# francescobrigante/Audio-Style-Transfer

Measured on AMD Instinct MI355X. Metric: audio-seconds/sec/node (train step, 4s@22.05kHz pairs), higher is better.
Workload: dtype bf16; 1 GPU; configs[1]: batch=8 4 s clips per GPU (S=2, x=(B,S,2,287,597)), full train2 step: STFT + CQT front-end from resident waveforms, encoders+decoder+discriminator, all losses, D and G phases, grad clip, Adam; global_batch=8, parallelism=dp1, hip_graph=True, dp_semantics=per-rank BN and batch-coupled losses

## Files before the change

### audio-style-transfer_amd/csrc/wgrad.hip

```cpp
#include "gemm_common.h"
#include <limits.h>

namespace {

#ifdef AST_STAMPS
__device__ unsigned long long ast_wg_stamps[4096 * 8];
__device__ long long ast_wg_phase[4096 * 4];
#define WG_STAMP(k) do { if (threadIdx.x == 0 && tix < 4096) ast_wg_stamps[tix * 8 + (k)] = (k) >= 6 ? wall_clock64() : __builtin_readcyclecounter(); } while (0)
#else
#define WG_STAMP(k) do { } while (0)
#endif
template <int BMW, int NCT, int RT, int CTW, typename WtOf>
__device__ __forceinline__ void flush_tile_rows(const f32x4 (&acc)[RT][CTW], float* tile, float* dw, const ast_gather_t& g, const int cd0,
                                                const int col0, const int ncols, const int wave, const int lane, WtOf wt_of, const int mode) {
  constexpr int BNW = NCT * 16;
  const int li = lane & 15, gq = lane >> 4;
  if (mode == 0) {
#pragma unroll
    for (int j = 0; j < CTW; ++j) {
      const int ct = wave + 4 * j;
      const int col = col0 + ct * 16 + li;
      if (ct >= NCT || col >= ncols) continue;
      const int t = col / g.Cs, c = col - t * g.Cs;
      const int wtc = wt_of(t);
#pragma unroll
      for (int i = 0; i < RT; ++i)
#pragma unroll
        for (int r = 0; r < 4; ++r) {
          const int cd = cd0 + i * 16 + gq * 4 + r;
          if (cd < g.Cd) unsafeAtomicAdd(dw + ((size_t)cd * g.wtaps + wtc) * g.Cs + c, acc[i][j][r]);
        }
    }
    return;
  }
  __syncthreads();
#pragma unroll
  for (int j = 0; j < CTW; ++j) {
    const int ct = wave + 4 * j;
    if (ct < NCT) {
#pragma unroll
      for (int i = 0; i < RT; ++i)
#pragma unroll
        for (int r = 0; r < 4; ++r) tile[(i * 16 + gq * 4 + r) * BNW + ct * 16 + li] = acc[i][j][r];
    }
  }
  __syncthreads();
#pragma unroll
  for (int cc = 0; cc < BNW / 64; ++cc) {
    const int col = col0 + cc * 64 + lane;
    if (col >= ncols) continue;
    const int t = col / g.Cs, c = col - t * g.Cs;
    float* dcol = dw + (size_t)wt_of(t) * g.Cs + c;
    if (mode == 2) {
      for (int row = wave; row < BMW; row += 4) {
        const int cd = cd0 + row;
        if (cd < g.Cd) dcol[(size_t)cd * g.wtaps * g.Cs] = tile[row * BNW + cc * 64 + lane];
      }
    } else {
      for (int row = wave; row < BMW; row += 4) {
        const int cd = cd0 + row;
        if (cd < g.Cd) unsafeAtomicAdd(dcol + (size_t)cd * g.wtaps * g.Cs, tile[row * BNW + cc * 64 + lane]);
      }
    }
  }
}

struct WgradFlush {
  enum Mode { Atomic = 0, AtomicLds = 1, Slab = 2 } mode;
  int copies;
  long stride;
  int* slices_out;
};
inline WgradFlush::Mode wg_atomic_mode() { return env_flag("AST_WGRAD_FLUSH_LDS", false) ? WgradFlush::AtomicLds : WgradFlush::Atomic; }
inline int wg_flush_arg(const WgradFlush& f) { return f.copies | ((int)f.mode << 16); }
inline int wg_slice_cap(const WgradFlush& f) { return f.mode == WgradFlush::Slab ? f.copies : INT_MAX; }
inline void wg_report_slices(const WgradFlush& f, int slices) { if (f.slices_out) *f.slices_out = slices; }
inline int wg_target_knob(int fallback) { return env_int("AST_WGRAD_WG_TARGET", fallback); }
inline int wg_pg_knob(int fallback) { return env_int("AST_WGRAD_PG", fallback); }

struct PixelSlices { int nsplit, pps, grid; };
inline PixelSlices plan_pixel_slices(int P, int k_unit, int min_trips, int tiles, int want, int cap) {
  const int min_px = min_trips * k_unit;
  int nsplit = std::min(std::max(1, std::min((P + min_px - 1) / min_px, want)), cap);
  int pps = (P + nsplit - 1) / nsplit;
  pps = (pps + k_unit - 1) / k_unit * k_unit;
  nsplit = (P + pps - 1) / pps;
  return {nsplit, pps, (tiles * nsplit + 7) / 8 * 8};
}
template <typename T> struct WgradCfg;
template <> struct WgradCfg<bf16_t> { static constexpr int BKP = 64, PAD = 16; };
template <> struct WgradCfg<float> { static constexpr int BKP = 32, PAD = 16; };

template <typename T, int BMW, int NCT, int PG, bool SLAB>
__global__ __launch_bounds__(256 * PG) void wgrad_kernel(const T* __restrict__ dy, const T* __restrict__ src,
                                                     float* __restrict__ dw, const ast_gather_t g,
                                                     const int P, const int pps, const unsigned dy_bytes,
                                                     const unsigned src_bytes, const float rcp_hw, const float rcp_w,
                                                     const int gx, const int gy, const int gz, const int nrep, const long rep_stride) {
  constexpr int E = 16 / sizeof(T), ES = sizeof(T);
  constexpr int BKP = WgradCfg<T>::BKP, PAD = WgradCfg<T>::PAD;
  constexpr int BNW = NCT * 16;
  constexpr int TPR = 256 / BKP;
  constexpr int CPX = BNW / E, CPY = BMW / E;
  constexpr int NXI = (CPX + TPR - 1) / TPR, NYI = (CPY + TPR - 1) / TPR;
  constexpr int PX = BNW + PAD, PY = BMW + PAD;
  constexpr bool SWZ = sizeof(T) == 2 && (CPX % 2 == 0) && (CPY % 2 == 0);
  constexpr int RT = BMW / 16;
  constexpr int CTW = (NCT + 3) / 4;
  constexpr unsigned OOB = 0x80000000u;
  extern __shared__ __attribute__((aligned(16))) unsigned char wl_all[];
  constexpr int GROUP_BYTES = (int)sizeof(T) * BKP * (PY + PX);
  constexpr int RED = PG > 1 ? RT * CTW * 256 * 16 : 0;
  constexpr int TILE = BMW * BNW * 4;
  constexpr int TAP_OFF = std::max(std::max(PG * GROUP_BYTES, RED), TILE);
  const int pg = PG > 1 ? __builtin_amdgcn_readfirstlane(threadIdx.x >> 8) : 0;
  unsigned char* wl = wl_all + pg * GROUP_BYTES;
  T* Ys = reinterpret_cast<T*>(wl);
  T* Xs = Ys + BKP * PY;
  int* taptab = reinterpret_cast<int*>(wl_all + TAP_OFF);

  const int tid = threadIdx.x & 255, lane = tid & 63, wave = tid >> 6;
  const int chunk = gridDim.x >> 3;
  const int tix = (blockIdx.x & 7) * chunk + (blockIdx.x >> 3);
  if (tix >= gx * gy * gz) return;
  WG_STAMP(0); WG_STAMP(7);
  const int bx = tix / (gz * gy), bz = (tix / gy) % gz, by = tix % gy;
  const int cd0 = bx * BMW, col0 = by * BNW;
  const int ncols = g.ntaps * g.Cs;
  const int HWm = g.Hm * g.Wm;
  const int p_begin = bz * pps, p_end = min(P, p_begin + pps);
  const __amdgpu_buffer_rsrc_t dyR = __builtin_amdgcn_make_buffer_rsrc((void*)dy, 0, dy_bytes, 0x00020000);
  const __amdgpu_buffer_rsrc_t srcR = __builtin_amdgcn_make_buffer_rsrc((void*)src, 0, src_bytes, 0x00020000);
#pragma unroll
  for (int t = 0; t < AST_MAX_TAPS; ++t)
    if ((int)threadIdx.x == t) taptab[t] = g.tap[t];
  __syncthreads();

  const int lrow = tid / TPR, tq = tid % TPR;
  int xdelta[NXI], xdh[NXI], xdw[NXI];
#pragma unroll
  for (int i = 0; i < NXI; ++i) {
    const int ch = tq + TPR * i, col = col0 + ch * E;
    xdelta[i] = 0; xdh[i] = 1 << 20; xdw[i] = 0;
    if (ch < CPX && col < ncols) {
      const int t = col / g.Cs, c = col - t * g.Cs;
      int dh, dw_, wt;
      decode_tap(taptab[t], dh, dw_, wt);
      xdh[i] = dh; xdw[i] = dw_;
      xdelta[i] = ((dh * g.Ws + dw_) * g.Cs + c) * ES;
    }
  }
  u32x4 yreg[NYI], xreg[NXI];
  auto load_tile = [&](int p0) __attribute__((always_inline)) {
    const int p = p0 + lrow;
    const bool pv = p < p_end;
    const int pp = pv ? p : 0;
#pragma unroll
    for (int i = 0; i < NYI; ++i) {
      const int ch = tq + TPR * i, cd = cd0 + ch * E;
      const bool ok = pv && ch < CPY && cd < g.Cd;
      yreg[i] = __builtin_amdgcn_raw_buffer_load_b128(dyR, ok ? (unsigned)((pp * g.Cd + cd) * ES) : OOB, 0, 0);
    }
    const int n = fdiv(pp, HWm, rcp_hw), rem = pp - n * HWm;
    const int hm = fdiv(rem, g.Wm, rcp_w), wq = rem - hm * g.Wm;
    const int hs0 = pv ? hm * g.sh + g.oh : -(1 << 21), ws0 = wq * g.sw + g.ow;
    const int base = (((n * g.Hs + hs0) * g.Ws + ws0) * g.Cs) * ES;
#pragma unroll
    for (int i = 0; i < NXI; ++i) {
      const bool ok = (unsigned)(hs0 + xdh[i]) < (unsigned)g.Hs && (unsigned)(ws0 + xdw[i]) < (unsigned)g.Ws;
      xreg[i] = __builtin_amdgcn_raw_buffer_load_b128(srcR, ok ? (unsigned)(base + xdelta[i]) : OOB, 0, 0);
    }
  };
  auto store_tile = [&]() __attribute__((always_inline)) {
    const int sw = SWZ ? ((lrow >> 3) & 1) << 1 : 0;
#pragma unroll
    for (int i = 0; i < NYI; ++i) {
      const int ch = tq + TPR * i;
      if (ch < CPY) *reinterpret_cast<u32x4*>(Ys + lrow * PY + (ch ^ sw) * E) = yreg[i];
    }
#pragma unroll
    for (int i = 0; i < NXI; ++i) {
      const int ch = tq + TPR * i;
      if (ch < CPX) *reinterpret_cast<u32x4*>(Xs + lrow * PX + (ch ^ sw) * E) = xreg[i];
    }
  };

  f32x4 acc[RT][CTW];
#pragma unroll
  for (int i = 0; i < RT; ++i)
#pragma unroll
    for (int j = 0; j < CTW; ++j) acc[i][j] = f32x4{0.f, 0.f, 0.f, 0.f};

  const int li = lane & 15, gq = lane >> 4;
  const int nk_all = (p_end - p_begin + BKP - 1) / BKP;
  const int nk = (nk_all + PG - 1) / PG;
  if (nk > 0) load_tile(p_begin + pg * BKP);
  WG_STAMP(1);
#ifdef AST_STAMPS
  long long ph[5] = {0, 0, 0, 0, 0};
#define WG_PH(i) do { const long long t_ = __builtin_readcyclecounter(); ph[i] += t_ - tph; tph = t_; } while (0)
  long long tph = __builtin_readcyclecounter();
#else
#define WG_PH(i) do { } while (0)
#endif
  for (int kt = 0; kt < nk; ++kt) {
    store_tile();
    WG_PH(0);
    __syncthreads();
    WG_PH(1);
    if (kt + 1 < nk) load_tile(p_begin + ((kt + 1) * PG + pg) * BKP);
    WG_PH(2);
    if constexpr (sizeof(T) == 2) {
      typedef __attribute__((address_space(3))) bf16x4 lds_b4;
      const int q = li >> 2, pcol = (li & 3) * 4;
#pragma unroll
      for (int ks = 0; ks < BKP / 32; ++ks) {
        const int r_lo = ks * 32 + 8 * gq + q;
        const int sx = SWZ ? (gq & 1) << 4 : 0;
        bf16x8 af[RT];
#pragma unroll
        for (int i = 0; i < RT; ++i) {
          const bf16x4 lo = __builtin_amdgcn_ds_read_tr16_b64_v4bf16((lds_b4*)(Ys + r_lo * PY + ((i * 16) ^ sx) + pcol));
          const bf16x4 hi = __builtin_amdgcn_ds_read_tr16_b64_v4bf16((lds_b4*)(Ys + (r_lo + 4) * PY + ((i * 16) ^ sx) + pcol));
          af[i] = bf16x8{lo[0], lo[1], lo[2], lo[3], hi[0], hi[1], hi[2], hi[3]};
        }
#pragma unroll
        for (int j = 0; j < CTW; ++j) {
          const int ct = wave + 4 * j;
          if (ct < NCT) {
            const bf16x4 lo = __builtin_amdgcn_ds_read_tr16_b64_v4bf16((lds_b4*)(Xs + r_lo * PX + ((ct * 16) ^ sx) + pcol));
            const bf16x4 hi = __builtin_amdgcn_ds_read_tr16_b64_v4bf16((lds_b4*)(Xs + (r_lo + 4) * PX + ((ct * 16) ^ sx) + pcol));
            const bf16x8 bf = bf16x8{lo[0], lo[1], lo[2], lo[3], hi[0], hi[1], hi[2], hi[3]};
#pragma unroll
            for (int i = 0; i < RT; ++i) acc[i][j] = __builtin_amdgcn_mfma_f32_16x16x32_bf16(af[i], bf, acc[i][j], 0, 0, 0);
          }
        }
      }
    } else {
#pragma unroll
      for (int s4 = 0; s4 < BKP / 4; ++s4) {
        float af[RT];
#pragma unroll
        for (int i = 0; i < RT; ++i) af[i] = Ys[(4 * s4 + gq) * PY + i * 16 + li];
#pragma unroll
        for (int j = 0; j < CTW; ++j) {
          const int ct = wave + 4 * j;
          if (ct < NCT) {
            const float bf = Xs[(4 * s4 + gq) * PX + ct * 16 + li];
#pragma unroll
            for (int i = 0; i < RT; ++i) acc[i][j] = __builtin_amdgcn_mfma_f32_16x16x4f32(af[i], bf, acc[i][j], 0, 0, 0);
          }
        }
      }
    }
    WG_PH(3);
    __syncthreads();
    WG_PH(4);
  }
#ifdef AST_STAMPS
  if (threadIdx.x == 0 && tix < 4096) { ast_wg_stamps[tix * 8 + 5] = (unsigned long long)((ph[0] << 32) | (ph[1] & 0xffffffffll)); ast_wg_phase[tix * 4 + 0] = ph[2]; ast_wg_phase[tix * 4 + 1] = ph[3]; ast_wg_phase[tix * 4 + 2] = ph[4]; ast_wg_phase[tix * 4 + 3] = nk; }
#endif

  WG_STAMP(2);
  if constexpr (PG > 1) {
    f32x4* red = reinterpret_cast<f32x4*>(wl_all);
#pragma unroll
    for (int src_g = 1; src_g < PG; ++src_g) {
      __syncthreads();
      if (pg == src_g) {
#pragma unroll
        for (int i = 0; i < RT; ++i)
#pragma unroll
          for (int j = 0; j < CTW; ++j) red[(i * CTW + j) * 256 + tid] = acc[i][j];
      }
      __syncthreads();
      if (pg == 0) {
#pragma unroll
        for (int i = 0; i < RT; ++i)
#pragma unroll
          for (int j = 0; j < CTW; ++j) {
            const f32x4 t = red[(i * CTW + j) * 256 + tid];
            acc[i][j][0] += t[0]; acc[i][j][1] += t[1]; acc[i][j][2] += t[2]; acc[i][j][3] += t[3];
          }
      }
    }
    if (pg > 0) return;
  }
  WG_STAMP(3);
  dw += (size_t)(bz % (nrep & 0xffff)) * rep_stride;
  flush_tile_rows<BMW, NCT, RT, CTW>(acc, reinterpret_cast<float*>(wl_all), dw, g, cd0, col0, ncols, wave, lane,
                                     [&](int t) { return taptab[t] >> 16; }, SLAB ? 2 : (nrep >> 16) & 3);
#ifdef AST_STAMPS
  asm volatile("s_waitcnt vmcnt(0)" ::: "memory");
#endif
  WG_STAMP(4); WG_STAMP(6);
}
#ifdef AST_STAMPS
extern "C" int ast_debug_read_wg_stamps(unsigned long long* host, int n) {
  return (int)hipMemcpyFromSymbol(host, HIP_SYMBOL(ast_wg_stamps), (size_t)n * 8 * sizeof(unsigned long long));
}
extern "C" int ast_debug_read_wg_phases(long long* host, int n) {
  return (int)hipMemcpyFromSymbol(host, HIP_SYMBOL(ast_wg_phase), (size_t)n * 4 * sizeof(long long));
}
// ... 406 lines not shown
#pragma unroll
        for (int i = 0; i < RT; ++i) {
          const bf16x4 lo = __builtin_amdgcn_ds_read_tr16_b64_v4bf16((lds_b4*)(Ys + p_lo * PY + i * 16 + pcol));
          const bf16x4 hi = __builtin_amdgcn_ds_read_tr16_b64_v4bf16((lds_b4*)(Ys + p_hi * PY + i * 16 + pcol));
          af[i] = bf16x8{lo[0], lo[1], lo[2], lo[3], hi[0], hi[1], hi[2], hi[3]};
        }
#pragma unroll
        for (int j = 0; j < CTW; ++j) {
          if (wave + 4 * j < NCT) {
            const bf16x4 lo = __builtin_amdgcn_ds_read_tr16_b64_v4bf16((lds_b4*)(Xp + x_lo + coloff[j]));
            const bf16x4 hi = __builtin_amdgcn_ds_read_tr16_b64_v4bf16((lds_b4*)(Xp + x_hi + coloff[j]));
            const bf16x8 bf = bf16x8{lo[0], lo[1], lo[2], lo[3], hi[0], hi[1], hi[2], hi[3]};
#pragma unroll
            for (int i = 0; i < RT; ++i) acc[i][j] = __builtin_amdgcn_mfma_f32_16x16x32_bf16(af[i], bf, acc[i][j], 0, 0, 0);
          }
        }
      }
    } else {
#pragma unroll 4
      for (int s4 = 0; s4 < MT / 4; ++s4) {
        const int p = 4 * s4 + gq;
        const int xo = (((p >> 4) * g.sh) * PW + (p & 15) * g.sw) * PPX;
        float af[RT];
#pragma unroll
        for (int i = 0; i < RT; ++i) af[i] = Ys[p * PY + i * 16 + li];
#pragma unroll
        for (int j = 0; j < CTW; ++j) {
          if (wave + 4 * j < NCT) {
            const float bf = colok[j] ? Xp[xo + coloff[j]] : 0.f;
#pragma unroll
            for (int i = 0; i < RT; ++i) acc[i][j] = __builtin_amdgcn_mfma_f32_16x16x4f32(af[i], bf, acc[i][j], 0, 0, 0);
          }
        }
      }
    }
    __syncthreads();
  }

  if constexpr (PG > 1) {
    f32x4* red = reinterpret_cast<f32x4*>(wl_all);
#pragma unroll
    for (int src_g = 1; src_g < PG; ++src_g) {
      __syncthreads();
      if (pg == src_g) {
#pragma unroll
        for (int i = 0; i < RT; ++i)
#pragma unroll
          for (int j = 0; j < CTW; ++j) red[(i * CTW + j) * 256 + tid] = acc[i][j];
      }
      __syncthreads();
      if (pg == 0) {
#pragma unroll
        for (int i = 0; i < RT; ++i)
#pragma unroll
          for (int j = 0; j < CTW; ++j) {
            const f32x4 t = red[(i * CTW + j) * 256 + tid];
            acc[i][j][0] += t[0]; acc[i][j][1] += t[1]; acc[i][j][2] += t[2]; acc[i][j][3] += t[3];
          }
      }
    }
    if (pg > 0) return;
  }
  dw += (size_t)(blockIdx.z % (nrep & 0xffff)) * rep_stride;
  flush_tile_rows<BMW, NCT, RT, CTW>(acc, reinterpret_cast<float*>(wl_all), dw, g, cd0, col0, ncols, wave, lane,
                                     [&](int t) { return taptab[16 + t]; }, SLAB ? 2 : (nrep >> 16) & 3);
}

bool plan_wgrad_halo(const ast_gather_t& g, int dtype, int nct, int bmw, WHaloPlan& hp) {
  if (g.ntaps < 2 || g.Cd > env_int("AST_WGRAD_HALO_MAXCD", 32)) return false;
  const int E = dtype == AST_BF16 ? 8 : 4, ES = dtype == AST_BF16 ? 2 : 4;
  int dhmin = 64, dhmax = -64, dwmin = 64, dwmax = -64;
  for (int t = 0; t < g.ntaps; ++t) {
    const int dh = (g.tap[t] & 255) - 64, dw = ((g.tap[t] >> 8) & 255) - 64;
    dhmin = std::min(dhmin, dh); dhmax = std::max(dhmax, dh); dwmin = std::min(dwmin, dw); dwmax = std::max(dwmax, dw);
  }
  hp.dhmin = dhmin; hp.dwmin = dwmin;
  hp.PH = (WH_TH - 1) * g.sh + (dhmax - dhmin) + 1;
  hp.PW = (WH_TW - 1) * g.sw + (dwmax - dwmin) + 1;
  if (hp.PH * hp.PW * (g.Cs / E) > 256 * WH_MAXPL) return false;
  hp.tiles_h = (g.Hm + WH_TH - 1) / WH_TH; hp.tiles_w = (g.Wm + WH_TW - 1) / WH_TW;
  hp.ntiles = g.N * hp.tiles_h * hp.tiles_w;
  const int ppx = g.Cs + (ES == 2 ? 8 : 4), pady = ES == 2 ? 8 : 16;
  hp.lds = ((ES * (WH_TH * WH_TW * (bmw + pady) + hp.PH * hp.PW * ppx) + 15) & ~15);
  if (hp.lds > 96 * 1024) return false;
  const double eff = (double)g.Hm * g.Wm / ((double)hp.tiles_h * hp.tiles_w * WH_TH * WH_TW);
  return eff >= 0.6 && hp.ntiles >= 256;
}

template <typename T, int BMW, int NCT, int PG>
int launch_wgrad_halo_pg(const void* dy, const void* src, float* dw, const ast_gather_t& g, const WHaloPlan& hp, const WgradFlush& f, hipStream_t s) {
  constexpr int RED = (BMW / 16) * ((NCT + 3) / 4) * 256 * 16;
  const int lds = std::max(std::max(PG * hp.lds, PG > 1 ? RED : 0), BMW * NCT * 16 * 4) + 160;
  static LdsAttrOnce attr;
  if (int rc = attr.set(160 * 1024, {(const void*)wgrad_halo_kernel<T, BMW, NCT, PG, false>, (const void*)wgrad_halo_kernel<T, BMW, NCT, PG, true>})) return rc;
  const int gx = (g.Cd + BMW - 1) / BMW, gy = (g.ntaps * g.Cs + NCT * 16 - 1) / (NCT * 16);
  const int wg_target = wg_target_knob(PG > 1 ? 256 : ((long)g.N * g.Hm * g.Wm >= 1500000 ? 768 : 256));
  const int gz = std::min(std::max(1, std::min((hp.ntiles + PG - 1) / PG, wg_target / (gx * gy))), wg_slice_cap(f));
  wg_report_slices(f, gz);
  const unsigned dy_bytes = (unsigned)((size_t)g.N * g.Hm * g.Wm * g.Cd * sizeof(T));
  const unsigned src_bytes = (unsigned)((size_t)g.N * g.Hs * g.Ws * g.Cs * sizeof(T));
  const auto k = f.mode == WgradFlush::Slab ? wgrad_halo_kernel<T, BMW, NCT, PG, true> : wgrad_halo_kernel<T, BMW, NCT, PG, false>;
  hipLaunchKernelGGL(k, dim3(gx, gy, gz), dim3(256 * PG), lds, s, (const T*)dy, (const T*)src, dw, g, hp, dy_bytes, src_bytes,
                     wg_flush_arg(f), f.stride);
  AST_CHECK_LAUNCH();
  return 0;
}

template <typename T, int BMW, int NCT>
int launch_wgrad_halo(const void* dy, const void* src, float* dw, const ast_gather_t& g, const WHaloPlan& hp, const WgradFlush& f, hipStream_t s) {
  int pg = wg_pg_knob(2);
  while (pg > 1 && (pg * hp.lds > 150 * 1024 || hp.ntiles < 256 * pg * 2)) pg >>= 1;
  if (pg >= 4) return launch_wgrad_halo_pg<T, BMW, NCT, 4>(dy, src, dw, g, hp, f, s);
  if (pg == 2) return launch_wgrad_halo_pg<T, BMW, NCT, 2>(dy, src, dw, g, hp, f, s);
  return launch_wgrad_halo_pg<T, BMW, NCT, 1>(dy, src, dw, g, hp, f, s);
}


template <typename T> struct WtCfg;
template <> struct WtCfg<bf16_t> { static constexpr int KPX = 32; };
template <> struct WtCfg<float> { static constexpr int KPX = 16; };

template <typename T, int NW>
__global__ __launch_bounds__(64 * NW) void wgrad_tap_kernel(const T* __restrict__ dy, const T* __restrict__ src, float* __restrict__ dw,
                                                            const ast_gather_t g, const int P, const int pps, const unsigned dy_bytes,
                                                            const unsigned src_bytes, const float rcp_hw, const float rcp_w, const int gx,
                                                            const int gy, const int gz, const int nrep, const long rep_stride, const int rmw) {
  constexpr int ES = sizeof(T), E = 16 / ES;
  constexpr int KPX = WtCfg<T>::KPX;
  constexpr int RB = 64 * ES;
  constexpr int CPR = RB / 16;
  constexpr int RPP = 64 / CPR;
  constexpr int NLD = KPX / RPP;
  constexpr int WAVE_LDS = 2 * KPX * RB;
  constexpr int RED_LDS = 64 * 64 * 4;
  constexpr int RPW = 64 / NW;
  constexpr unsigned OOB = 0x80000000u;
  static_assert(64 % NW == 0 && NLD == 4 && WAVE_LDS <= RED_LDS, "tile");
  extern __shared__ __attribute__((aligned(16))) unsigned char wt_lds[];
  int* taptab = reinterpret_cast<int*>(wt_lds + NW * RED_LDS);

  const int lane = threadIdx.x & 63;
  const int wave = __builtin_amdgcn_readfirstlane(threadIdx.x >> 6);
  const int chunk = gridDim.x >> 3;
  const int tix = (blockIdx.x & 7) * chunk + (blockIdx.x >> 3);
  const int tiles = gx * gy;
  if (tix >= tiles * gz) return;
  const int bz = tix / tiles, tile = tix - bz * tiles;
  const int bx = tile / gy, by = tile - bx * gy;
  const int cd0 = bx * 64, col0 = by * 64;
  const int ncols = g.ntaps * g.Cs;
  const int HWm = g.Hm * g.Wm;
  const int p_begin = bz * pps, p_end = min(P, p_begin + pps);
  if (p_begin >= p_end) return;
  const __amdgpu_buffer_rsrc_t dyR = __builtin_amdgcn_make_buffer_rsrc((void*)dy, 0, dy_bytes, 0x00020000);
  const __amdgpu_buffer_rsrc_t srcR = __builtin_amdgcn_make_buffer_rsrc((void*)src, 0, src_bytes, 0x00020000);
#pragma unroll
  for (int t = 0; t < AST_MAX_TAPS; ++t)
    if ((int)threadIdx.x == t) taptab[t] = g.tap[t];
  __syncthreads();

  const int c = lane % CPR, r0 = lane / CPR;
  const int cdc = cd0 + c * E;
  const bool yok = cdc < g.Cd;
  const int colc = col0 + c * E;
  const bool xok = colc < ncols;
  int xdh = 0, xdw = 0, xdelta = 0;
  {
    const int t = xok ? colc / g.Cs : 0, ch = xok ? colc - t * g.Cs : 0;
    int wt;
    decode_tap(taptab[t], xdh, xdw, wt);
    xdelta = ((xdh * g.Ws + xdw) * g.Cs + ch) * ES;
  }
  int lofs[NLD];
#pragma unroll
  for (int i = 0; i < NLD; ++i) {
    const int r = r0 + i * RPP;
    if constexpr (ES == 2) lofs[i] = r * RB + ((((c >> 1) ^ (((r >> 1) & 1) | (((r >> 3) & 1) << 1))) << 5) | ((c & 1) << 4));
    else lofs[i] = r * RB + ((((c >> 2) ^ (r & 1)) << 6) | ((c & 3) << 4));
  }
  unsigned char* Yw = wt_lds + wave * WAVE_LDS;
  unsigned char* Xw = Yw + KPX * RB;

  u32x4 yreg[NLD], xreg[NLD];
  auto load_step = [&](int ks) __attribute__((always_inline)) {
    const int pb = p_begin + ks * KPX + r0;
#pragma unroll
    for (int i = 0; i < NLD; ++i) {
      const int p = pb + i * RPP;
      const bool pv = p < p_end;
      const int pp = pv ? p : 0;
      yreg[i] = __builtin_amdgcn_raw_buffer_load_b128(dyR, (pv && yok) ? (unsigned)((pp * g.Cd + cdc) * ES) : OOB, 0, 0);
      const int n = fdiv(pp, HWm, rcp_hw), rem = pp - n * HWm;
      const int hm = fdiv(rem, g.Wm, rcp_w), wq = rem - hm * g.Wm;
      const int hs0 = hm * g.sh + g.oh, ws0 = wq * g.sw + g.ow;
      const bool ok = pv && xok && (unsigned)(hs0 + xdh) < (unsigned)g.Hs && (unsigned)(ws0 + xdw) < (unsigned)g.Ws;
      xreg[i] = __builtin_amdgcn_raw_buffer_load_b128(srcR, ok ? (unsigned)((((n * g.Hs + hs0) * g.Ws + ws0) * g.Cs) * ES + xdelta) : OOB, 0, 0);
    }
  };

  f32x4 acc[4][4];
#pragma unroll
  for (int i = 0; i < 4; ++i)
#pragma unroll
    for (int j = 0; j < 4; ++j) acc[i][j] = f32x4{0.f, 0.f, 0.f, 0.f};

  const int li = lane & 15, gq = lane >> 4;
  const int nks = (p_end - p_begin + KPX - 1) / KPX;
  int ks = wave;
  if (ks < nks) load_step(ks);
  for (; ks < nks; ks += NW) {
#pragma unroll
    for (int i = 0; i < NLD; ++i) {
      *reinterpret_cast<u32x4*>(Yw + lofs[i]) = yreg[i];
      *reinterpret_cast<u32x4*>(Xw + lofs[i]) = xreg[i];
    }
    asm volatile("" ::: "memory");
    if (ks + NW < nks) load_step(ks + NW);
    if constexpr (ES == 2) {
      typedef __attribute__((address_space(3))) bf16x4 lds_b4;
      const int r_lo = 8 * gq + (li >> 2), r_hi = r_lo + 4;
      const int g_lo = ((r_lo >> 1) & 1) | (((r_lo >> 3) & 1) << 1), g_hi = ((r_hi >> 1) & 1) | (((r_hi >> 3) & 1) << 1);
      const int b_lo = r_lo * RB + (li & 3) * 8, b_hi = r_hi * RB + (li & 3) * 8;
      bf16x8 af[4];
#pragma unroll
      for (int i = 0; i < 4; ++i) {
        const bf16x4 lo = __builtin_amdgcn_ds_read_tr16_b64_v4bf16((lds_b4*)(Yw + b_lo + ((i ^ g_lo) << 5)));
        const bf16x4 hi = __builtin_amdgcn_ds_read_tr16_b64_v4bf16((lds_b4*)(Yw + b_hi + ((i ^ g_hi) << 5)));
        af[i] = bf16x8{lo[0], lo[1], lo[2], lo[3], hi[0], hi[1], hi[2], hi[3]};
      }
#pragma unroll
      for (int j = 0; j < 4; ++j) {
        const bf16x4 lo = __builtin_amdgcn_ds_read_tr16_b64_v4bf16((lds_b4*)(Xw + b_lo + ((j ^ g_lo) << 5)));
        const bf16x4 hi = __builtin_amdgcn_ds_read_tr16_b64_v4bf16((lds_b4*)(Xw + b_hi + ((j ^ g_hi) << 5)));
        const bf16x8 bf = bf16x8{lo[0], lo[1], lo[2], lo[3], hi[0], hi[1], hi[2], hi[3]};
#pragma unroll
        for (int i = 0; i < 4; ++i) acc[i][j] = __builtin_amdgcn_mfma_f32_16x16x32_bf16(af[i], bf, acc[i][j], 0, 0, 0);
      }
    } else {
#pragma unroll
      for (int s4 = 0; s4 < KPX / 4; ++s4) {
        const int r = 4 * s4 + gq;
        const int base = r * RB + li * 4;
        float af[4];
#pragma unroll
        for (int i = 0; i < 4; ++i) af[i] = *reinterpret_cast<const float*>(Yw + base + ((i ^ (r & 1)) << 6));
#pragma unroll
        for (int j = 0; j < 4; ++j) {
          const float bf = *reinterpret_cast<const float*>(Xw + base + ((j ^ (r & 1)) << 6));
#pragma unroll
          for (int i = 0; i < 4; ++i) acc[i][j] = __builtin_amdgcn_mfma_f32_16x16x4f32(af[i], bf, acc[i][j], 0, 0, 0);
        }
      }
    }
    asm volatile("" ::: "memory");
  }

  __syncthreads();
  float* red = reinterpret_cast<float*>(wt_lds) + wave * (64 * 64);
#pragma unroll
  for (int i = 0; i < 4; ++i)
#pragma unroll
    for (int j = 0; j < 4; ++j)
#pragma unroll
      for (int r = 0; r < 4; ++r) red[(16 * i + 4 * gq + r) * 64 + 16 * j + li] = acc[i][j][r];
  __syncthreads();
  const int col = col0 + lane;
  const bool cok = col < ncols;
  const int t = cok ? col / g.Cs : 0, ch = cok ? col - t * g.Cs : 0;
  const int wtc = taptab[t] >> 16;
  float* dwr = dw + (size_t)(bz % nrep) * rep_stride;
  const float* rbase = reinterpret_cast<const float*>(wt_lds);
#pragma unroll
  for (int rr = 0; rr < RPW; ++rr) {
    const int row = RPW * wave + rr, cd = cd0 + row;
    float v = 0.f;
#pragma unroll
    for (int w = 0; w < NW; ++w) v += rbase[w * (64 * 64) + row * 64 + lane];
    if (cok && cd < g.Cd) {
      float* dst = dwr + ((size_t)cd * g.wtaps + wtc) * g.Cs + ch;
      if (rmw) *dst += v;
      else unsafeAtomicAdd(dst, v);
    }
  }
}

template <typename T>
int launch_wgrad_tap(const void* dy, const void* src, float* dw, const ast_gather_t& g, int P, const WgradFlush& f, hipStream_t s) {
  constexpr int NW = 8, KPX = WtCfg<T>::KPX;
  constexpr int LDS = NW * 64 * 64 * 4 + 64;
  static LdsAttrOnce attr;
  if (int rc = attr.set(LDS, {(const void*)wgrad_tap_kernel<T, NW>})) return rc;
  const int gx = (g.Cd + 63) / 64, gy = (g.ntaps * g.Cs + 63) / 64, tiles = gx * gy;
  const int wg_target = env_int("AST_WGRAD_TAP_WGS", 256);
  const PixelSlices ps = plan_pixel_slices(P, KPX, 2 * NW, tiles, (wg_target + tiles / 2) / tiles, wg_slice_cap(f));
  const unsigned dy_bytes = (unsigned)((size_t)P * g.Cd * sizeof(T));
  const unsigned src_bytes = (unsigned)((size_t)g.N * g.Hs * g.Ws * g.Cs * sizeof(T));
  wg_report_slices(f, ps.nsplit);
  hipLaunchKernelGGL((wgrad_tap_kernel<T, NW>), dim3(ps.grid), dim3(64 * NW), LDS, s, (const T*)dy, (const T*)src, dw, g, P, ps.pps, dy_bytes, src_bytes,
                     1.0f / (float)(g.Hm * g.Wm), 1.0f / (float)g.Wm, gx, gy, ps.nsplit, f.copies, f.stride, ps.nsplit == 1 ? 1 : 0);
  AST_CHECK_LAUNCH();
  return 0;
}

int wgrad_dispatch(const void* dy, const void* src, float* dw, const ast_gather_t* gp, int dtype, const WgradFlush& f, hipStream_t s) {
  if (int rc = check_gather(gp, "ast_wgrad")) return rc;
  if (!dy || !src || !dw) AST_FAIL("ast_wgrad: null pointer");
  const ast_gather_t g = *gp;
  if (g.ntaps == 0) return 0;
  const int P = g.N * g.Hm * g.Wm;
  if ((long)P * g.Cd * 4 >= (1L << 31)) AST_FAIL("ast_wgrad: dy exceeds the 2 GiB buffer-addressing range");
  const int nct_all = (g.ntaps * g.Cs + 15) / 16;
  const int bmw = g.Cd > 32 ? 64 : (g.Cd > 16 ? 32 : 16);
  int nct;
  if (bmw == 64) nct = nct_all <= 8 ? (nct_all <= 4 ? 4 : 8) : 12;
  else nct = nct_all <= 4 ? 4 : (nct_all <= 8 ? 8 : (nct_all <= 12 ? 12 : 20));
  if (env_flag("AST_WGRAD_TAP", false) && f.mode != WgradFlush::Slab && g.Cd >= 64) {
    AST_DISPATCH_T(dtype, { return launch_wgrad_tap<T>(dy, src, dw, g, P, f, s); });
  }
  if (env_flag("AST_WGRAD_ROWS", true) && wgrad_rows_eligible(g, dtype)) {
    if ((long)P * g.Cs * 2 >= (1L << 31)) AST_FAIL("ast_wgrad: source exceeds the 2 GiB buffer-addressing range");
    const int nst = env_int("AST_WGRAD_ROWS_STAGES", 4);
    if (nst == 2) return launch_wgrad_rows<2>(dy, src, dw, g, P, f, s);
    if (nst == 3) return launch_wgrad_rows<3>(dy, src, dw, g, P, f, s);
    return launch_wgrad_rows<4>(dy, src, dw, g, P, f, s);
  }
  WHaloPlan whp;
  const bool halo = plan_wgrad_halo(g, dtype, nct, bmw, whp);
#define AST_WG(B_, N_) do { if (halo) return launch_wgrad_halo<T, B_, N_>(dy, src, dw, g, whp, f, s); \
                            return launch_wgrad<T, B_, N_>(dy, src, dw, g, P, f, s); } while (0)
  AST_DISPATCH_T(dtype, {
    if (bmw == 64) { if (nct == 4) AST_WG(64, 4); if (nct == 8) AST_WG(64, 8); AST_WG(64, 12); }
    if (bmw == 32) { if (nct == 4) AST_WG(32, 4); if (nct == 8) AST_WG(32, 8); if (nct == 12) AST_WG(32, 12); AST_WG(32, 20); }
    if (nct == 4) AST_WG(16, 4); if (nct == 8) AST_WG(16, 8); if (nct == 12) AST_WG(16, 12); AST_WG(16, 20);
  });
#undef AST_WG
  return 0;
}

}

extern "C" int ast_wgrad(const void* dy, const void* src, float* dw, const ast_gather_t* gp, int dtype, void* stream) {
  return wgrad_dispatch(dy, src, dw, gp, dtype, WgradFlush{wg_atomic_mode(), 1, 0, nullptr}, (hipStream_t)stream);
}

extern "C" int ast_wgrad_rep(const void* dy, const void* src, float* dw, const ast_gather_t* gp, int dtype, int nrep, void* stream) {
  if (nrep < 1 || nrep > 64 || !gp) AST_FAIL("ast_wgrad_rep: 1..64 replicas");
  return wgrad_dispatch(dy, src, dw, gp, dtype, WgradFlush{wg_atomic_mode(), nrep, (long)gp->Cd * gp->wtaps * gp->Cs, nullptr}, (hipStream_t)stream);
}

namespace {
struct SlabRec { float* base; unsigned n, slabs; };
struct SlabArgs { SlabRec rec[AST_MAX_SLAB_RECS]; unsigned first_block[AST_MAX_SLAB_RECS + 1]; int nrec; };
__global__ __launch_bounds__(256) void slab_sum_kernel(const SlabArgs a) {
  int r = 0;
#pragma unroll 1
  while (r + 1 < a.nrec && blockIdx.x >= a.first_block[r + 1]) ++r;
  float* base = nullptr; unsigned n = 0, slabs = 0, fb = 0;
#pragma unroll
  for (int i = 0; i < AST_MAX_SLAB_RECS; ++i)
    if (i == r) { base = a.rec[i].base; n = a.rec[i].n; slabs = a.rec[i].slabs; fb = a.first_block[i]; }
  const unsigned i4 = ((blockIdx.x - fb) * 256 + threadIdx.x) * 4;
  if (i4 >= n) return;
  f32x4 acc = *reinterpret_cast<const f32x4*>(base + i4);
  unsigned s = 1;
  for (; s + 8 <= slabs; s += 8) {
    f32x4 t[8];
#pragma unroll
    for (int k = 0; k < 8; ++k) t[k] = *reinterpret_cast<const f32x4*>(base + (size_t)(s + k) * n + i4);
    acc += ((t[0] + t[1]) + (t[2] + t[3])) + ((t[4] + t[5]) + (t[6] + t[7]));
  }
  for (; s < slabs; ++s) acc += *reinterpret_cast<const f32x4*>(base + (size_t)s * n + i4);
  *reinterpret_cast<f32x4*>(base + i4) = acc;
}
}

extern "C" int ast_wgrad_slab(const void* dy, const void* src, float* slabs, const ast_gather_t* gp, int dtype, int nslabs, int* slices_out,
                              void* stream) {
  if (nslabs < 1 || nslabs > 4096 || !gp || !slices_out) AST_FAIL("ast_wgrad_slab: 1..4096 slabs and a slices output");
  *slices_out = 0;
  return wgrad_dispatch(dy, src, slabs, gp, dtype, WgradFlush{WgradFlush::Slab, nslabs, (long)gp->Cd * gp->wtaps * gp->Cs, slices_out}, (hipStream_t)stream);
}

extern "C" int ast_slab_sum(float* const* bases, const int64_t* floats_per_copy, const int* slabs, int nrec, void* stream) {
  if (!bases || !floats_per_copy || !slabs || nrec < 1 || nrec > AST_MAX_SLAB_RECS) AST_FAIL("ast_slab_sum: 1..%d records", AST_MAX_SLAB_RECS);
  SlabArgs a;
  unsigned blocks = 0;
  a.nrec = nrec;
  for (int i = 0; i < AST_MAX_SLAB_RECS; ++i) {
    a.rec[i] = SlabRec{nullptr, 0, 0};
    a.first_block[i] = blocks;
    if (i < nrec) {
      if (!bases[i] || floats_per_copy[i] < 4 || (floats_per_copy[i] & 3) || floats_per_copy[i] > (1L << 30) || slabs[i] < 1 || (((uintptr_t)bases[i]) & 15))
        AST_FAIL("ast_slab_sum: record %d: 16-byte aligned base, a multiple of 4 floats per copy, >= 1 copies", i);
      a.rec[i] = SlabRec{bases[i], (unsigned)floats_per_copy[i], (unsigned)slabs[i]};
      blocks += (unsigned)((floats_per_copy[i] + 1023) / 1024);
    }
  }
  a.first_block[AST_MAX_SLAB_RECS] = blocks;
  hipLaunchKernelGGL(slab_sum_kernel, dim3(blocks), dim3(256), 0, (hipStream_t)stream, a);
  AST_CHECK_LAUNCH();
  return 0;
}
```

Before: 5281 audio-seconds/sec.

## Add narrow-channel wgrad kernel with sliding row window for small Cd/Cs convs

Adds a specialized weight-gradient kernel for bf16 convolutions with at most 32 output channels and 8/16/32 input channels, 1x1 or 3x3 taps, stride 1 or 2. Each wave walks a run of output rows in a 64-pixel segment and keeps a rolling window of KS input rows in LDS, so each input row is loaded once and reused across vertical taps. Loads for the next row are register-prefetched while MFMAs run on the current one. Per-wave accumulators are reduced in LDS and flushed with atomics or slab writes. It is enabled by default for large enough pixel counts and adds planning heuristics and many template instantiations, with some risk of atomic contention and low occupancy from the large LDS footprint.

```diff
diff --git a/audio-style-transfer_amd/csrc/wgrad.hip b/audio-style-transfer_amd/csrc/wgrad.hip
--- a/audio-style-transfer_amd/csrc/wgrad.hip
+++ b/audio-style-transfer_amd/csrc/wgrad.hip
@@ -1,4 +1,5 @@
 #include "gemm_common.h"
+#include "wgrad_narrow_plan.h"
 #include <limits.h>
 
 namespace {
@@ -1011,6 +1012,225 @@
   return 0;
 }
 
+struct WNarrowArgs { int nseg, segw, nrb, nruns, dh0, dw0; };
+
+template <int CD, int CS, int KS, int S, bool SLAB>
+__global__ __launch_bounds__(64 * NARROW_NW) void wgrad_narrow_kernel(const bf16_t* __restrict__ dy, const bf16_t* __restrict__ src,
+                                                                       float* __restrict__ dw, const ast_gather_t g, const WNarrowArgs a,
+                                                                       const unsigned dy_bytes, const unsigned src_bytes, const int copies,
+                                                                       const long rep_stride) {
+  constexpr int SEG = NARROW_SEG, NW = NARROW_NW;
+  constexpr int PY = CD + 8, PPX = CS + 8;
+  constexpr int XW = (SEG - 1) * S + KS;
+  constexpr int CPY = CD / 8, UP = CS / 8;
+  constexpr int NY = SEG * CPY / 64;
+  constexpr int NX = (XW * UP + 63) / 64;
+  constexpr int NEW = KS == 1 ? 1 : S;
+  constexpr int PRO = KS - NEW;
+  constexpr int RT = CD / 16, NCOL = KS * KS * CS, NCT = (NCOL + 15) / 16, BN = NCT * 16;
+  constexpr int YB = SEG * PY * 2, XB = XW * PPX * 2;
+  constexpr int WAVE_LDS = (YB + KS * XB + 15) & ~15;
+  constexpr int TILE = CD * BN * 4;
+  constexpr unsigned OOB = 0x80000000u;
+  static_assert(NEW <= KS && (YB & 15) == 0 && (XB & 15) == 0, "window");
+  typedef __attribute__((address_space(3))) bf16x4 lds_b4;
+  extern __shared__ __attribute__((aligned(16))) unsigned char wn_lds[];
+  int* taptab = reinterpret_cast<int*>(wn_lds + (NW * WAVE_LDS > TILE ? NW * WAVE_LDS : TILE));
+
+  const int lane = threadIdx.x & 63;
+  const int wave = __builtin_amdgcn_readfirstlane(threadIdx.x >> 6);
+  const __amdgpu_buffer_rsrc_t dyR = __builtin_amdgcn_make_buffer_rsrc((void*)dy, 0, dy_bytes, 0x00020000);
+  const __amdgpu_buffer_rsrc_t srcR = __builtin_amdgcn_make_buffer_rsrc((void*)src, 0, src_bytes, 0x00020000);
+#pragma unroll
+  for (int t = 0; t < AST_MAX_TAPS; ++t)
+    if ((int)threadIdx.x == t) taptab[t] = g.tap[t] >> 16;
+  __syncthreads();
+
+  unsigned char* Yw = wn_lds + wave * WAVE_LDS;
+  unsigned char* Xw = Yw + YB;
+
+  int ypx[NY], ych[NY], xpx[NX], xpart[NX];
+#pragma unroll
+  for (int i = 0; i < NY; ++i) { const int idx = lane + 64 * i; ypx[i] = idx / CPY; ych[i] = idx % CPY; }
+#pragma unroll
+  for (int j = 0; j < NX; ++j) { const int idx = lane + 64 * j; xpx[j] = idx / UP; xpart[j] = idx % UP; }
+
+  const int li = lane & 15, gq = lane >> 4;
+  const int prow = 8 * gq + (li >> 2), pcol = (li & 3) * 4;
+  int xcol[NCT], xkh[NCT];
+#pragma unroll
+  for (int j = 0; j < NCT; ++j) {
+    int t, c;
+    if constexpr (CS >= 16) { t = (16 * j) / CS; c = (16 * j) % CS + pcol; }
+    else { const int col = 16 * j + pcol; t = col / CS; c = col % CS; }
+    if (t >= KS * KS) { t = 0; c = 0; }
+    xkh[j] = t / KS;
+    xcol[j] = ((t % KS) * PPX + c) * 2 + prow * S * PPX * 2;
+  }
+  const int yrow = prow * PY * 2 + pcol * 2;
+
+  f32x4 acc[RT][NCT];
+#pragma unroll
+  for (int i = 0; i < RT; ++i)
+#pragma unroll
+    for (int j = 0; j < NCT; ++j) acc[i][j] = f32x4{0.f, 0.f, 0.f, 0.f};
+
+  const int rstep = gridDim.x * NW;
+  for (int run = blockIdx.x * NW + wave; run < a.nruns; run += rstep) {
+    const int seg = run % a.nseg, tq = run / a.nseg;
+    const int rb = tq % a.nrb, n = tq / a.nrb;
+    const int h0 = (int)((long)rb * g.Hm / a.nrb), nrows = (int)((long)(rb + 1) * g.Hm / a.nrb) - h0;
+    const int w0 = seg * a.segw, segn = min(a.segw, g.Wm - w0);
+    const int hs0 = h0 * S + g.oh + a.dh0, ws0 = w0 * S + g.ow + a.dw0;
+    const int xneed = (segn - 1) * S + KS;
+    int ybase = ((n * g.Hm + h0) * g.Wm + w0) * g.Cd * 2;
+    const int ystride = g.Wm * g.Cd * 2, xstride = g.Ws * g.Cs * 2;
+    int yoff[NY], xoff[NX];
+    bool yok[NY], xok[NX];
+#pragma unroll
+    for (int i = 0; i < NY; ++i) {
+      yok[i] = ypx[i] < segn && ych[i] * 8 < g.Cd;
+      yoff[i] = (ypx[i] * g.Cd + ych[i] * 8) * 2;
+    }
+#pragma unroll
+    for (int j = 0; j < NX; ++j) {
+      xok[j] = xpx[j] < xneed && (unsigned)(ws0 + xpx[j]) < (unsigned)g.Ws;
+      xoff[j] = ((ws0 + xpx[j]) * g.Cs + xpart[j] * 8) * 2;
+    }
+    u32x4 yreg[NY], xreg[NEW][NX];
+    auto load_x = [&](u32x4 (&r)[NX], int hs) __attribute__((always_inline)) {
+      const bool rowok = (unsigned)hs < (unsigned)g.Hs;
+      const int rbase = (n * g.Hs + (rowok ? hs : 0)) * xstride;
+#pragma unroll
+      for (int j = 0; j < NX; ++j) r[j] = __builtin_amdgcn_raw_buffer_load_b128(srcR, (rowok && xok[j]) ? (unsigned)(rbase + xoff[j]) : OOB, 0, 0);
+    };
+    auto store_x = [&](const u32x4 (&r)[NX], int slot) __attribute__((always_inline)) {
+#pragma unroll
+      for (int j = 0; j < NX; ++j)
+        if (xpx[j] < XW) *reinterpret_cast<u32x4*>(Xw + slot * XB + (xpx[j] * PPX + xpart[j] * 8) * 2) = r[j];
+    };
+    auto load_step = [&](int i) __attribute__((always_inline)) {
+#pragma unroll
+      for (int k = 0; k < NY; ++k) yreg[k] = __builtin_amdgcn_raw_buffer_load_b128(dyR, yok[k] ? (unsigned)(ybase + yoff[k]) : OOB, 0, 0);
+      ybase += ystride;
+#pragma unroll
+      for (int k = 0; k < NEW; ++k) load_x(xreg[k], hs0 + i * S + PRO + k);
+    };
+
+    asm volatile("" ::: "memory");
+    if constexpr (PRO > 0) {
+      u32x4 xpro[PRO][NX];
+#pragma unroll
+      for (int r = 0; r < PRO; ++r) load_x(xpro[r], hs0 + r);
+      load_step(0);
+#pragma unroll
+      for (int r = 0; r < PRO; ++r) store_x(xpro[r], r);
+    } else {
+      load_step(0);
+    }
+    int rb3 = 0;
+    for (int i = 0; i < nrows; ++i) {
+#pragma unroll
+      for (int k = 0; k < NY; ++k) *reinterpret_cast<u32x4*>(Yw + (ypx[k] * PY + ych[k] * 8) * 2) = yreg[k];
+#pragma unroll
+      for (int k = 0; k < NEW; ++k) {
+        int slot = rb3 + PRO + k;
+        slot = KS == 1 ? 0 : (slot >= 2 * KS ? slot - 2 * KS : (slot >= KS ? slot - KS : slot));
+        store_x(xreg[k], slot);
+      }
+      asm volatile("" ::: "memory");
+      if (i + 1 < nrows) load_step(i + 1);
+      int xrow[NCT];
+#pragma unroll
+      for (int j = 0; j < NCT; ++j) {
+        int slot = rb3 + xkh[j];
+        slot = KS == 1 ? 0 : (slot >= KS ? slot - KS : slot);
+        xrow[j] = slot * XB + xcol[j];
+      }
+#pragma unroll
+      for (int ks = 0; ks < SEG / 32; ++ks) {
+        if (ks * 32 < segn) {
+          bf16x8 af[RT];
+#pragma unroll
+          for (int r = 0; r < RT; ++r) {
+            const bf16x4 lo = __builtin_amdgcn_ds_read_tr16_b64_v4bf16((lds_b4*)(Yw + yrow + ks * 32 * PY * 2 + r * 32));
+            const bf16x4 hi = __builtin_amdgcn_ds_read_tr16_b64_v4bf16((lds_b4*)(Yw + yrow + (ks * 32 + 4) * PY * 2 + r * 32));
+            af[r] = bf16x8{lo[0], lo[1], lo[2], lo[3], hi[0], hi[1], hi[2], hi[3]};
+          }
+#pragma unroll
+          for (int j = 0; j < NCT; ++j) {
+            const bf16x4 lo = __builtin_amdgcn_ds_read_tr16_b64_v4bf16((lds_b4*)(Xw + xrow[j] + ks * 32 * S * PPX * 2));
+            const bf16x4 hi = __builtin_amdgcn_ds_read_tr16_b64_v4bf16((lds_b4*)(Xw + xrow[j] + (ks * 32 + 4) * S * PPX * 2));
+            const bf16x8 bf = bf16x8{lo[0], lo[1], lo[2], lo[3], hi[0], hi[1], hi[2], hi[3]};
+#pragma unroll
+            for (int r = 0; r < RT; ++r) acc[r][j] = __builtin_amdgcn_mfma_f32_16x16x32_bf16(af[r], bf, acc[r][j], 0, 0, 0);
+          }
+        }
+      }
+      asm volatile("" ::: "memory");
+      rb3 += NEW;
+      if (rb3 >= KS) rb3 -= KS;
+    }
+  }
+
+  float* tile = reinterpret_cast<float*>(wn_lds);
+#pragma unroll 1
+  for (int w = 0; w < NW; ++w) {
+    __syncthreads();
+    if (wave == w) {
+#pragma unroll
+      for (int r = 0; r < RT; ++r)
+#pragma unroll
+        for (int j = 0; j < NCT; ++j)
+#pragma unroll
+          for (int e = 0; e < 4; ++e) {
+            float* p = tile + (16 * r + 4 * gq + e) * BN + 16 * j + li;
+            *p = w == 0 ? acc[r][j][e] : *p + acc[r][j][e];
+          }
+    }
+  }
+  __syncthreads();
+  float* dwc = dw + (size_t)(SLAB ? blockIdx.x : blockIdx.x % copies) * rep_stride;
+  for (int e = threadIdx.x; e < CD * NCOL; e += 64 * NW) {
+    const int row = e / NCOL, col = e - row * NCOL;
+    if (row >= g.Cd) break;
+    const int t = col / CS, c = col - t * CS;
+    float* dst = dwc + ((size_t)row * g.wtaps + taptab[t]) * g.Cs + c;
+    const float v = tile[row * BN + col];
+    if constexpr (SLAB) *dst = v; else unsafeAtomicAdd(dst, v);
+  }
+}
+
+#define AST_NARROW_KERNELS(CD_, CS_, KS_, S_) {(const void*)wgrad_narrow_kernel<CD_, CS_, KS_, S_, false>, (const void*)wgrad_narrow_kernel<CD_, CS_, KS_, S_, true>}
+template <int CD, int CS, int KS, int S>
+int launch_wgrad_narrow_t(const void* dy, const void* src, float* dw, const ast_gather_t& g, const WNarrowPlan& np, const WgradFlush& f, hipStream_t s) {
+  static LdsAttrOnce attr;
+  if (int rc = attr.set(NARROW_LDS_LIMIT, AST_NARROW_KERNELS(CD, CS, KS, S))) return rc;
+  const WNarrowArgs a{np.nseg, np.segw, np.nrb, np.nruns, np.dh0, np.dw0};
+  const unsigned dy_bytes = (unsigned)((size_t)g.N * g.Hm * g.Wm * g.Cd * 2);
+  const unsigned src_bytes = (unsigned)((size_t)g.N * g.Hs * g.Ws * g.Cs * 2);
+  wg_report_slices(f, np.grid);
+  const auto k = f.mode == WgradFlush::Slab ? wgrad_narrow_kernel<CD, CS, KS, S, true> : wgrad_narrow_kernel<CD, CS, KS, S, false>;
+  hipLaunchKernelGGL(k, dim3(np.grid), dim3(64 * NARROW_NW), np.lds, s, (const bf16_t*)dy, (const bf16_t*)src, dw, g, a, dy_bytes, src_bytes,
+                     std::max(1, f.copies), f.stride);
+  AST_CHECK_LAUNCH();
+  return 0;
+}
+#undef AST_NARROW_KERNELS
+
+int launch_wgrad_narrow(const void* dy, const void* src, float* dw, const ast_gather_t& g, const WNarrowPlan& np, const WgradFlush& f, hipStream_t s) {
+  if (f.mode == WgradFlush::Slab && np.grid > wg_slice_cap(f)) AST_FAIL("ast_wgrad: narrow plan of %d slices for %d slab copies", np.grid, f.copies);
+  if (np.lds > NARROW_LDS_LIMIT || np.grid < 1) AST_FAIL("ast_wgrad: bad narrow plan (%d bytes of LDS, grid %d)", np.lds, np.grid);
+#define AST_WN(CD_, CS_, KS_, S_) if (np.cd_t == CD_ && np.cs_t == CS_ && np.ks == KS_ && np.stride == S_) \
+    return launch_wgrad_narrow_t<CD_, CS_, KS_, S_>(dy, src, dw, g, np, f, s)
+#define AST_WN_CD(CS_, KS_, S_) AST_WN(16, CS_, KS_, S_); AST_WN(32, CS_, KS_, S_)
+  AST_WN_CD(8, 3, 1); AST_WN_CD(16, 3, 1); AST_WN_CD(32, 3, 1); AST_WN_CD(8, 3, 2); AST_WN_CD(16, 3, 2);
+  AST_WN_CD(8, 1, 1); AST_WN_CD(16, 1, 1); AST_WN_CD(32, 1, 1); AST_WN_CD(8, 1, 2); AST_WN_CD(16, 1, 2); AST_WN_CD(32, 1, 2);
+#undef AST_WN_CD
+#undef AST_WN
+  AST_FAIL("ast_wgrad: no narrow kernel for Cd %d, Cs %d, %d taps, stride %d", np.cd_t, np.cs_t, np.ks * np.ks, np.stride);
+}
+
 int wgrad_dispatch(const void* dy, const void* src, float* dw, const ast_gather_t* gp, int dtype, const WgradFlush& f, hipStream_t s) {
   if (int rc = check_gather(gp, "ast_wgrad")) return rc;
   if (!dy || !src || !dw) AST_FAIL("ast_wgrad: null pointer");
@@ -1033,6 +1253,11 @@
     if (nst == 3) return launch_wgrad_rows<3>(dy, src, dw, g, P, f, s);
     return launch_wgrad_rows<4>(dy, src, dw, g, P, f, s);
   }
+  WNarrowPlan wnp;
+  if (plan_wgrad_narrow(g, dtype, wgrad_narrow_mode(), f.mode == WgradFlush::Slab, wg_slice_cap(f), f.copies, wnp)) {
+    if ((long)g.N * g.Hs * g.Ws * g.Cs * 2 >= (1L << 31)) AST_FAIL("ast_wgrad: source exceeds the 2 GiB buffer-addressing range");
+    return launch_wgrad_narrow(dy, src, dw, g, wnp, f, s);
+  }
   WHaloPlan whp;
   const bool halo = plan_wgrad_halo(g, dtype, nct, bmw, whp);
 #define AST_WG(B_, N_) do { if (halo) return launch_wgrad_halo<T, B_, N_>(dy, src, dw, g, whp, f, s); \
diff --git a/audio-style-transfer_amd/csrc/wgrad_narrow_plan.h b/audio-style-transfer_amd/csrc/wgrad_narrow_plan.h
--- /dev/null
+++ b/audio-style-transfer_amd/csrc/wgrad_narrow_plan.h
@@ -0,0 +1,65 @@
+#pragma once
+#include <limits.h>
+#include <stdlib.h>
+#include <algorithm>
+#include "../../include/ast_hip.h"
+
+constexpr int NARROW_SEG = 64;
+constexpr int NARROW_NW = 4;
+constexpr int NARROW_LDS_LIMIT = 160 * 1024;
+constexpr int NARROW_CUS = 256;
+
+struct WNarrowPlan {
+  int ks, stride, cd_t, cs_t;
+  int dh0, dw0;
+  int nseg, segw;
+  int nrb;
+  int nruns;
+  int grid;
+  int wave_lds, lds;
+};
+
+inline int wgrad_narrow_mode() { const char* e = getenv("AST_WGRAD_NARROW"); return e ? atoi(e) : 1; }
+
+inline long env_narrow_min_pixels() { const char* e = getenv("AST_WGRAD_NARROW_MINP"); return e ? atol(e) : 100000; }
+
+inline int wgrad_narrow_wave_lds(int ks, int stride, int cd_t, int cs_t) {
+  return (2 * (NARROW_SEG * (cd_t + 8) + ks * ((NARROW_SEG - 1) * stride + ks) * (cs_t + 8)) + 15) & ~15;
+}
+
+inline bool plan_wgrad_narrow(const ast_gather_t& g, int dtype, int mode, bool slab, int slice_cap, int copies, WNarrowPlan& np) {
+  if (mode <= 0 || dtype != AST_DTYPE_BF16) return false;
+  if (g.Cd > 32 || (g.Cs != 8 && g.Cs != 16 && g.Cs != 32)) return false;
+  if (g.sh != g.sw || (g.sh != 1 && g.sh != 2)) return false;
+  const int ks = g.ntaps == 9 ? 3 : (g.ntaps == 1 ? 1 : 0);
+  if (!ks) return false;
+  const int dh0 = (g.tap[0] & 255) - 64, dw0 = ((g.tap[0] >> 8) & 255) - 64;
+  for (int t = 0; t < g.ntaps; ++t)
+    if ((g.tap[t] & 255) - 64 != dh0 + t / ks || ((g.tap[t] >> 8) & 255) - 64 != dw0 + t % ks) return false;
+  if (ks == 3 && g.sh == 2 && g.Cs == 32) return false;
+  const long P = (long)g.N * g.Hm * g.Wm;
+  if (mode == 1 && P < env_narrow_min_pixels()) return false;
+  if (mode == 1 && ks == 3 && g.Cd > 16) return false;
+  np.ks = ks; np.stride = g.sh; np.cd_t = g.Cd > 16 ? 32 : 16; np.cs_t = g.Cs; np.dh0 = dh0; np.dw0 = dw0;
+  np.wave_lds = wgrad_narrow_wave_lds(ks, g.sh, np.cd_t, np.cs_t);
+  const int nct = (ks * ks * np.cs_t + 15) / 16;
+  np.lds = std::max(NARROW_NW * np.wave_lds, np.cd_t * nct * 16 * 4) + 64;
+  if (np.lds > NARROW_LDS_LIMIT) return false;
+  np.nseg = (g.Wm + NARROW_SEG - 1) / NARROW_SEG;
+  np.segw = (g.Wm + np.nseg - 1) / np.nseg;
+  const int per_cu = std::max(1, std::min(4, NARROW_LDS_LIMIT / np.lds));
+  int wgs = NARROW_CUS * per_cu;
+  if (slab) wgs = std::min(wgs, slice_cap);
+  else wgs = std::min(wgs, std::max(NARROW_CUS, 128 * std::max(1, copies)));
+  { const char* e = getenv("AST_WGRAD_NARROW_WGS"); if (e && atoi(e) > 0) wgs = std::min(atoi(e), slab ? slice_cap : INT_MAX); }
+  wgs = std::max(1, wgs);
+  const long cols = (long)g.N * np.nseg;
+  const int max_rb = std::max(1, g.Hm / 4);
+  np.nrb = (int)std::min<long>(max_rb, std::max<long>(1, ((long)wgs * NARROW_NW + cols - 1) / cols));
+  const long nruns = cols * np.nrb;
+  if (nruns >= (1L << 30)) return false;
+  np.nruns = (int)nruns;
+  np.grid = (int)std::min<long>(wgs, (nruns + NARROW_NW - 1) / NARROW_NW);
+  if (mode == 1 && slab && np.grid < NARROW_CUS) return false;
+  return true;
+}
```

Result: no change. 5330 audio-seconds/sec (median of 6 runs) (+0.9%).
